# CMU-Quake/hercules

Hardware: AMD Instinct MI355X
Metric: element-updates/sec (whole node) + achieved HBM GB/s, 64M-elem box (higher is better)
Workload: dtype f64

## Files before the change

hercules_amd/capi.py:

```python
import ctypes
import os

import numpy as np

_HERE = os.path.dirname(os.path.abspath(__file__))
_LIBPATH = os.environ.get("HQ_SOLVER_LIB") or os.path.join(_HERE, "csrc", "libhq_solver.so")

HQ_VARIANT_AUTO, HQ_VARIANT_SCATTER, HQ_VARIANT_PATCH = 0, 1, 2
IPC_BLOB_BYTES = 4096

EXPORTS = ["hq_device_count", "hq_last_error", "hq_create", "hq_destroy", "hq_get_info", "hq_get_info_sized", "hq_abi_version", "hq_comm_init_ipc_n",
           "hq_options_init", "hq_create_opts", "hq_get_options", "hq_real_bytes",
           "hq_comm_unique_id", "hq_comm_init", "hq_comm_selftest", "hq_group_link", "hq_group_run", "hq_set_source", "hq_run", "hq_sync", "hq_gather", "hq_gather3",
           "hq_download", "hq_upload", "hq_phase_force", "hq_phase_update", "hq_download_force",
           "hq_run_timed", "hq_dominant_kernel", "hq_plan_check", "hq_stencil_plan_check", "hq_check_finite",
           "hq_stencil_coefficients", "hq_brick_plan_check", "hq_brick_plan_check_n", "hq_comm_init_host",
           "hq_comm_ipc_export", "hq_comm_init_ipc", "hq_comm_init_loopback",
           "hq_record_add", "hq_record_pending", "hq_record_fetch", "hq_record_clear",
           "hq_snapshot_add", "hq_snapshot_pending", "hq_snapshot_fetch", "hq_snapshot_clear",
           "hq_peak_add", "hq_peak_fetch", "hq_peak_load", "hq_peak_reset", "hq_peak_clear",
           "hq_spec_add", "hq_spec_coefficients", "hq_spec_fetch", "hq_spec_load", "hq_spec_reset", "hq_spec_clear",
           "hq_cum_add", "hq_cum_fetch", "hq_cum_load", "hq_cum_reset", "hq_cum_clear"]
HQ_SNAP_TM1, HQ_SNAP_TM2, HQ_SNAP_VEL = 1, 2, 4
HQ_PEAK_DISP, HQ_PEAK_VEL, HQ_PEAK_ACC = 1, 2, 4
HQ_SPEC_MAX_PERIODS, HQ_SPEC_NVAL = 32, 4


class HqError(RuntimeError):
    pass


HOST_EXCHANGE_FN = ctypes.CFUNCTYPE(ctypes.c_int, ctypes.c_void_p, ctypes.c_int32, ctypes.POINTER(ctypes.c_int32),
                                    ctypes.POINTER(ctypes.c_int64), ctypes.POINTER(ctypes.c_void_p), ctypes.c_int32,
                                    ctypes.POINTER(ctypes.c_int32), ctypes.POINTER(ctypes.c_int64),
                                    ctypes.POINTER(ctypes.c_void_p), ctypes.c_int32)


class _Messenger(ctypes.Structure):
    _fields_ = [("procid", ctypes.c_int32), ("nodecount", ctypes.c_int32),
                ("mapping", ctypes.c_void_p)]


class _Schedule(ctypes.Structure):
    _fields_ = [("c_count", ctypes.c_int32), ("first_c", ctypes.POINTER(_Messenger)),
                ("s_count", ctypes.c_int32), ("first_s", ctypes.POINTER(_Messenger))]


class _Desc(ctypes.Structure):
    _fields_ = [("lenum", ctypes.c_int32), ("nharbored", ctypes.c_int32), ("ldnnum", ctypes.c_int32),
# ... 37 lines not shown
                ("quantities", ctypes.c_int32), ("husid_every", ctypes.c_int32), ("husid_slots", ctypes.c_int32),
                ("reserved", ctypes.c_int32), ("threshold", ctypes.c_double * 3)]


class _Info(ctypes.Structure):
    _fields_ = [("variant", ctypes.c_int32), ("npatches", ctypes.c_int32),
                ("patch_pairs", ctypes.c_int64), ("device_bytes", ctypes.c_int64),
                ("step", ctypes.c_int32), ("nranks", ctypes.c_int32),
                ("lattice_patches", ctypes.c_int32), ("stencil_patches", ctypes.c_int32),
                ("ragged_patches", ctypes.c_int32), ("brick_units", ctypes.c_int32),
                ("brick_nodes", ctypes.c_int64), ("brick_units_pernode", ctypes.c_int32),
                ("brick_units_het", ctypes.c_int32), ("pcie_h2d_bytes", ctypes.c_int64),
                ("pcie_d2h_bytes", ctypes.c_int64), ("transport", ctypes.c_int32), ("ipc_arena_coarse", ctypes.c_int32),
                ("ipc_arena_kind", ctypes.c_int32), ("debug_halo", ctypes.c_int32),
                ("brick_units_packed", ctypes.c_int32), ("brick_units_ragged", ctypes.c_int32),
                ("brick_stream", ctypes.c_int32), ("brick_units_ragged_het", ctypes.c_int32), ("timed_steps", ctypes.c_int64),
                ("t_step_us", ctypes.c_double), ("t_shell_us", ctypes.c_double), ("t_interior_us", ctypes.c_double),
                ("t_chain_us", ctypes.c_double), ("t_chain_exposed_us", ctypes.c_double)]


OPTION_FIELDS = ["no_bricks", "brick_cz", "brick_minz", "brick_minnodes", "brick_no_het", "brick_no_ntsame", "brick_by_component",
                 "brick_stream", "brick_no_faces", "brick_half_tiles", "brick_no_pack", "patch_pipe", "patch_threads", "patch_pmax", "patch_pmerge", "patch_psplit", "patch_nlmax",
                 "patch_vmax", "patch_ragged", "patch_no_lattice", "patch_no_stencil", "patch_no_uniform", "patch_no_iso",
                 "patch_no_ntsame", "patch_no_dedup", "patch_wform", "patch_merge_rounds", "overlap", "no_overlap", "reserve_cus",
                 "cu_mask", "no_fused_share", "group_copies", "debug_halo", "ipc_arena"]


class Options(ctypes.Structure):
    _fields_ = ([("size", ctypes.c_uint64)] + [(n, ctypes.c_int32) for n in OPTION_FIELDS] +
                [("ipc_timeout_ms", ctypes.c_double), ("loopback_delay_us", ctypes.c_double),
                 ("verbose", ctypes.c_int32), ("quiet", ctypes.c_int32),
                 ("brick_ragged", ctypes.c_int32), ("brick_ragged_minfill", ctypes.c_int32),
                 ("allow_env", ctypes.c_int32), ("brick_ragged_het", ctypes.c_int32), ("reserved0", ctypes.c_int32),
                 ("phase_timing", ctypes.c_int32)])

    def __init__(self, **kw):
        super().__init__()
        load_library().hq_options_init(ctypes.byref(self), ctypes.c_uint64(ctypes.sizeof(self)))
        for k, v in kw.items():
            if k not in dict(self._fields_):
                raise TypeError("hq_options has no field %r" % k)
            setattr(self, k, v)

    def as_dict(self):
        return {k: getattr(self, k) for k, _ in self._fields_ if k != "size"}


_lib = None
_lib_f32 = None
_LIBPATH_F32 = os.environ.get("HQ_SOLVER_LIB_F32") or os.path.join(_HERE, "csrc", "libhq_solver_f32.so")


def load_library(path=None, precision="f64"):
    global _lib, _lib_f32
    if precision == "f32" and path is None:
        if _lib_f32 is None:
            _lib_f32 = load_library(_LIBPATH_F32)
            if _lib_f32.hq_real_bytes() != 4:
                raise HqError("%s was not built with -DHQ_SINGLE_PRECISION_SOLVER" % _LIBPATH_F32)
        return _lib_f32
    if _lib is not None and path is None:
        return _lib
    p = path or _LIBPATH
    if not os.path.exists(p):
        raise HqError("native library %s is missing: run `python -m hercules_amd.build` "
                      "(there is no Python/CPU fallback)" % p)
    probe = ctypes.CDLL(p, mode=ctypes.RTLD_LOCAL)
# ... 428 lines not shown
        return f


PLAN_REPORT = ("patches", "lattice_patches", "pairs", "distinct_row_blocks", "gather_passes", "gather_instructions",
               "lattice_gather_passes", "faults")


def plan_check(desc):
    rep = (ctypes.c_int64 * 8)()
    _check(load_library().hq_plan_check(ctypes.byref(desc), rep))
    return dict(zip(PLAN_REPORT, [int(v) for v in rep]))


STENCIL_PLAN_REPORT = ("patches", "tables", "full_lattices", "boundary_nodes", "corners_checked", "faults")


def stencil_plan_check(desc):
    rep = (ctypes.c_int64 * 6)()
    _check(load_library().hq_stencil_plan_check(ctypes.byref(desc), rep))
    return dict(zip(STENCIL_PLAN_REPORT, [int(v) for v in rep]))


BRICK_PLAN_REPORT = ("brick_nodes", "columns", "units", "units_one_nt_row", "het_units", "neighbours_checked",
                     "patch_nodes", "faults", "ragged_units", "ragged_nodes", "ragged_het_units", "ragged_het_nodes", "packed_units",
                     "min_unit_nx", "min_unit_ny", "min_unit_np", "ragged_min_plane_nodes", "units_one_plane_both_faces")


def brick_plan_check(desc):
    rep = (ctypes.c_int64 * len(BRICK_PLAN_REPORT))()
    _check(load_library().hq_brick_plan_check_n(ctypes.byref(desc), rep, ctypes.c_int32(len(BRICK_PLAN_REPORT))))
    return dict(zip(BRICK_PLAN_REPORT, [int(v) for v in rep]))


def comm_unique_id():
    buf = (ctypes.c_char * 128)()
    _check(load_library().hq_comm_unique_id(buf))
    return bytes(buf)


def group_link(solvers):
    arr = (ctypes.c_void_p * len(solvers))(*[s._h for s in solvers])
    lib = solvers[0]._lib
    _check(lib.hq_group_link(arr, ctypes.c_int32(len(solvers))), lib)


def group_run(solvers, nsteps):
    arr = (ctypes.c_void_p * len(solvers))(*[s._h for s in solvers])
    lib = solvers[0]._lib
    _check(lib.hq_group_run(arr, ctypes.c_int32(len(solvers)), ctypes.c_int32(nsteps)), lib)
    for s in solvers:
        s.sync()
```

hercules_amd/csrc/hq_brick.h:

```cpp
#ifndef HQ_BRICK_H
#define HQ_BRICK_H

#include <chrono>
#include <map>

#include "hq_patch.h"

#define HQ_BK_TX 64
#ifndef HQ_BK_TY
#define HQ_BK_TY 8
#endif
#define HQ_BK_THREADS (HQ_BK_TX * HQ_BK_TY)
#define HQ_BK_PY (HQ_BK_TX + 2)
#define HQ_BK_PLANE ((HQ_BK_TX + 2) * (HQ_BK_TY + 2))
#ifndef HQ_BK_ATTR
#define HQ_BK_ATTR
#endif
#define HQ_BK_NTSAME 1
#define HQ_BK_HET 2
#define HQ_BK_TOPFACE 8
#define HQ_BK_BOTFACE 16
#define HQ_BK_RAGGED 32
#define HQ_BK_PACKED 4
#ifndef HQ_BH_WAVES
#define HQ_BH_WAVES 8
#endif
#define HQ_BH_THREADS (64 * HQ_BH_WAVES)
#define HQ_BH_NRT (64 + 2 * (HQ_BH_WAVES - 1))
#define HQ_BH_TX 62
#define HQ_BH_TY (HQ_BH_WAVES - 1)
#define HQ_BH_PY 65
#define HQ_BH_CS HQ_BH_THREADS
#define HQ_BH_ROWS (65 * (HQ_BH_WAVES + 1))

struct hq_brick_unit {
    int64_t base;
    int64_t tab;
    int32_t nx, ny, np, flags;
    double  c1, c2, beta;
    double  m0, m2, m1;
    double  ft[7], fb[7];
    int64_t coef;
};

struct hq_brick_cfg {
    int cz = 32;
    int minz = 4;
    int minnodes = 512;
    int ragged = 1;
// ... 425 lines not shown
                    }
        }
        if (twice) { g_patch_err = "brick plan: a node lies in two tile columns"; return -1; }
    }
    {
        int nth = 1;
#pragma omp parallel
        {
#pragma omp single
            nth = omp_get_num_threads();
        }
        std::vector<int64_t> first((size_t)nth + 1, 0);
#pragma omp parallel for schedule(static, 1)
        for (int t = 0; t < nth; t++) {
            const int64_t lo = N * t / nth, hi = N * (t + 1) / nth;
            int64_t cnt = 0;
            for (int64_t n = lo; n < hi; n++) cnt += B->perm[(size_t)n] < 0;
            first[(size_t)t + 1] = cnt;
        }
        for (int i = 0; i < nth; i++) first[(size_t)i + 1] += first[(size_t)i];
#pragma omp parallel for schedule(static, 1)
        for (int t = 0; t < nth; t++) {
            const int64_t lo = N * t / nth, hi = N * (t + 1) / nth;
            int64_t k = nb + first[(size_t)t];
            for (int64_t n = lo; n < hi; n++) if (B->perm[(size_t)n] < 0) B->perm[(size_t)n] = (int32_t)k++;
        }
        if (nb + first[(size_t)nth] != N) { g_patch_err = "brick plan: numbering is not a permutation"; return -1; }
    }
    lap("numbering");
    B->nb = nb;
    B->ncolumns = (int32_t)cols.size();
    B->nlevels = (int32_t)levels.size();

    struct unit_t { int col; int32_t za, np; int64_t key; };
    std::vector<unit_t> us;
    int cz = cfg.cz;
    if (!hq_given(o.brick_cz)) {
        for (cz = 32; cz > 8; cz /= 2) {
            int64_t n = 0;
            for (auto& c : cols) n += (c.nz + cz - 1) / cz;
            if (n >= 512) break;
        }
    }
    for (size_t ci = 0; ci < cols.size(); ci++) {
        const column_t& c = cols[ci];
        const int32_t nch = (c.nz + cz - 1) / cz;
        const int32_t G = std::max(1, 64 / std::max(1, ntx_of_level[(size_t)c.lvl]));
        for (int32_t k = 0; k < nch; k++) {
            const int32_t za = (int32_t)((int64_t)c.nz * k / nch), zb = (int32_t)((int64_t)c.nz * (k + 1) / nch);
            const int64_t key = ((int64_t)c.lvl << 56) | ((int64_t)(c.tj / G) << 42) | ((int64_t)((c.z0 + za) / cz) << 28) |
                                ((int64_t)(c.tj % G) << 20) | (int64_t)c.ti;
            us.push_back({ (int)ci, c.z0 + za, zb - za, key });
        }
    }
    std::stable_sort(us.begin(), us.end(), [](const unit_t& a, const unit_t& b) { return a.key < b.key; });
    B->units.resize(us.size());
    std::vector<int64_t> toff(us.size() + 1, 0);
    for (size_t u = 0; u < us.size(); u++) {
        const column_t& c = cols[(size_t)us[u].col];
        const int64_t nr = 2 * (c.nx + 2) + 2 * c.ny;
        toff[u + 1] = toff[u] + ((int64_t)(us[u].np + 2) * nr + (c.rag ? us[u].np + 2 : 2) * (int64_t)c.nx * c.ny + 3) / 4 * 4;
    }
    B->tab.assign((size_t)toff[us.size()] + 64, 0);
    std::vector<int64_t> coff(us.size() + 1, 0);
    for (size_t u = 0; u < us.size(); u++)
        coff[u + 1] = coff[u] + (cols[(size_t)us[u].col].het ? (int64_t)(us[u].np + 1) * HQ_BH_THREADS * 3 : 0);
    B->coef.assign((size_t)coff[us.size()] + 8, 0.0);
    const bool try_pack = MS && MS->edata && MS->dt > 0 && !hq_set(o.brick_no_pack);
    if (try_pack) { B->coef32.assign((size_t)coff[us.size()] + 8, 0.0f); B->nt2.assign(2 * (size_t)N, 0.0); }
    int fault = 0;
    auto set_fault = [&]() {
#pragma omp atomic write
        fault = 1;
    };
    std::vector<char> same(us.size(), 0);
#pragma omp parallel for schedule(dynamic, 16)
    for (int64_t u = 0; u < (int64_t)us.size(); u++) {
        const column_t& c = cols[(size_t)us[(size_t)u].col];
        const level_t& L = levels[(size_t)c.lvl];
        const int64_t NX = L.D[0] + 1, NY = L.D[1] + 1;
        const int32_t za = us[(size_t)u].za, np = us[(size_t)u].np, nx = c.nx, ny = c.ny, nr = 2 * (nx + 2) + 2 * ny;
        auto dev = [&](int64_t X, int64_t Y, int64_t Z) -> int32_t {
            if (X < 0 || Y < 0 || Z < 0 || X > L.D[0] || Y > L.D[1] || Z > L.D[2]) { set_fault(); return 0; }
            const int32_t n = L.Ng[(size_t)((Z * NY + Y) * NX + X)];
            if (n < 0) { set_fault(); return 0; }
            return B->perm[(size_t)n];
        };
        int32_t* t = B->tab.data() + toff[(size_t)u];
// ... 202 lines not shown
    return __hiloint2double(hi, lo);
}

template <bool PERNODE, bool BYCOMP, bool RAGGED = false>
__global__ void HQ_BK_ATTR __launch_bounds__(HQ_BK_THREADS, 4)
hq_k_brick(int32_t count, int32_t per_xcd, const hq_brick_unit* __restrict__ units, const int32_t* __restrict__ tab,
           const hq_real* __restrict__ u1g, const hq_real* __restrict__ u2g, hq_real* __restrict__ ung,
           const double* __restrict__ nt3, const int32_t* __restrict__ src_ptr, const int32_t* __restrict__ src_ent,
           const double* __restrict__ F, double dt2, hq_stencil_coef sc)
{
    __shared__ __align__(16) double s_w[2 * 3 * HQ_BK_PLANE];
    const int slot = (int)(blockIdx.x & 7) * per_xcd + (int)(blockIdx.x >> 3);
    if (slot >= count) return;
    const hq_brick_unit U = units[slot];
    const int nx = U.nx, ny = U.ny, np = U.np, nxy = nx * ny, nr = 2 * (nx + 2) + 2 * ny;
    const int t = threadIdx.x, lx = t & (HQ_BK_TX - 1), ly = t >> 6;
    const bool active = lx < nx && ly < ny;
    const int sidx = active ? ly * nx + lx : 0;
    const int myrow = (ly + 1) * HQ_BK_PY + lx + 1;
    const bool ring = t < nr;
    int rrow;
    {
        int rx, ry;
        if (t < nx + 2) { rx = t - 1; ry = -1; }
        else if (t < 2 * (nx + 2)) { rx = t - (nx + 2) - 1; ry = ny; }
        else if (t < 2 * (nx + 2) + ny) { rx = -1; ry = t - 2 * (nx + 2); }
        else { rx = nx; ry = t - 2 * (nx + 2) - ny; }
        rrow = (ry + 1) * HQ_BK_PY + rx + 1;
    }
    const int32_t* __restrict__ utab = tab + U.tab;
    const int rofs = ring ? t : 0;
    const int32_t* __restrict__ cap = utab + (int64_t)(np + 2) * nr;
    int32_t vOut = -1, vMid = RAGGED ? cap[sidx] : 0, vCur = RAGGED ? cap[nxy + sidx] : 0, vNext = 0;
    const int32_t id_lo = RAGGED ? (vMid >= 0 ? vMid : -vMid - 2) : cap[sidx];
    const double beta = U.beta;
    double P[6], Q[2];
#pragma unroll
    for (int i = 0; i < 6; i++) P[i] = hq_uniform(U.c1 * sc.p1[i] + U.c2 * sc.p2[i]);
#pragma unroll
    for (int i = 0; i < 2; i++) Q[i] = hq_uniform(U.c1 * sc.q1[i] + U.c2 * sc.q2[i]);
    const bool has_src = F && src_ptr[slot + 1] > src_ptr[slot];

    hq_real x1[3] = { 0, 0, 0 }, x2[3] = { 0, 0, 0 }, y1[3] = { 0, 0, 0 }, y2[3] = { 0, 0, 0 };
    double mn[3] = { U.m0, U.m2, U.m1 };
    double m0A = hq_uniform(1.0 / U.m0), m0B = m0A;
    double fA[3] = { 0.0, 0.0, 0.0 }, fB[3] = { 0.0, 0.0, 0.0 };
    int32_t rid = utab[rofs];

#define HQ_BK_LOAD(node_)                                                                             \
    {                                                                                                 \
        const int64_t a_ = (node_);                                                                   \
        if (active && (!RAGGED || a_ >= 0)) {                                                         \
            _Pragma("unroll") for (int d = 0; d < 3; d++) { x1[d] = u1g[3 * a_ + d]; x2[d] = u2g[3 * a_ + d]; } \
            if (PERNODE) { _Pragma("unroll") for (int d = 0; d < 3; d++) mn[d] = nt3[3 * a_ + d]; }    \
        }                                                                                             \
        if (ring && (!RAGGED || rid >= 0)) {                                                          \
            const int64_t b_ = (int64_t)rid;                                                          \
            _Pragma("unroll") for (int d = 0; d < 3; d++) { y1[d] = u1g[3 * b_ + d]; y2[d] = u2g[3 * b_ + d]; } \
        }                                                                                             \
    }
#define HQ_BK_PUT(s_, acc_, M2_, M1_)                                                                 \
    {                                                                                                 \
        hq_lds_double* img_ = (hq_lds_double*)s_w + 3 * HQ_BK_PLANE * (s_);                            \
        if (active) {                                                                                 \
            _Pragma("unroll") for (int d = 0; d < 3; d++) {                                           \
                const double a1_ = x1[d], a2_ = x2[d];                                                \
                img_[3 * myrow + d] = a1_ + beta * (a1_ - a2_);                                       \
                acc_[d] += (M2_) * a1_ - (M1_) * a2_;                                                 \
            }                                                                                         \
        }                                                                                             \
        if (ring) { _Pragma("unroll") for (int d = 0; d < 3; d++) { const double b1_ = y1[d], b2_ = y2[d]; img_[3 * rrow + d] = b1_ + beta * (b1_ - b2_); } } \
    }

    const bool topf = !PERNODE && !RAGGED && (U.flags & HQ_BK_TOPFACE) != 0, botf = !PERNODE && !RAGGED && (U.flags & HQ_BK_BOTFACE) != 0;
    const double rho = hq_uniform((U.c1 - U.c2) / (U.c1 + U.c2));

    HQ_BK_LOAD((int64_t)id_lo)
    rid = utab[nr + rofs];
    if (topf) HQ_BK_PUT(0, fB, U.ft[1 + d], U.ft[4 + d])
    else { double dummy[3] = { 0.0, 0.0, 0.0 }; HQ_BK_PUT(0, dummy, mn[1], mn[2]) }
    for (int k = 0; k <= np + 1; k++) {
        if (k <= np) {
            if (RAGGED) {
                HQ_BK_LOAD((int64_t)(vCur >= 0 ? vCur : -vCur - 2))
                if (k < np) vNext = cap[(k + 2) * nxy + sidx];
            } else HQ_BK_LOAD(k == np ? (int64_t)cap[nxy + sidx] : U.base + (int64_t)k * nxy + sidx)
            if (k < np) rid = utab[(k + 2) * nr + rofs];
        }
        __syncthreads();
        const hq_lds_double* __restrict__ q = (const hq_lds_double*)s_w + 3 * (HQ_BK_PLANE * (k & 1) + myrow);
        double m[3], g[3], Uo[3];
        if (BYCOMP) {
            double A_x, A_y;
            {
                const double C = q[2], XM = q[2 - 3], XP = q[2 + 3], YM = q[2 - 3 * HQ_BK_PY], YP = q[2 + 3 * HQ_BK_PY];
                const double MM = q[2 - 3 * HQ_BK_PY - 3], PM = q[2 - 3 * HQ_BK_PY + 3], MP = q[2 + 3 * HQ_BK_PY - 3], PP = q[2 + 3 * HQ_BK_PY + 3];
                const double sxy = (XM + XP) + (YM + YP), dg = (MM + PP) + (PM + MP);
                m[2] = fma(P[0], C, fma(P[2], sxy, P[4] * dg));
                g[2] = fma(P[1], C, fma(P[3], sxy, P[5] * dg));
                Uo[0] = fma(Q[0], XP - XM, Q[1] * ((PP - MP) + (PM - MM)));
                Uo[1] = fma(Q[0], YP - YM, Q[1] * ((PP - PM) + (MP - MM)));
            }
            __builtin_amdgcn_sched_barrier(0);
            {
                const double C = q[0], XM = q[0 - 3], XP = q[0 + 3], YM = q[0 - 3 * HQ_BK_PY], YP = q[0 + 3 * HQ_BK_PY];
                const double MM = q[0 - 3 * HQ_BK_PY - 3], PM = q[0 - 3 * HQ_BK_PY + 3], MP = q[0 + 3 * HQ_BK_PY - 3], PP = q[0 + 3 * HQ_BK_PY + 3];
                const double sx = XM + XP, sy = YM + YP, dg = (MM + PP) + (PM + MP);
                A_x = (PP + MM) - (PM + MP);
                m[0] = fma(P[0], C, fma(P[1], sx, fma(P[2], sy, P[3] * dg)));
                g[0] = fma(P[2], C, fma(P[3], sx, fma(P[4], sy, P[5] * dg)));
                Uo[2] = fma(Q[0], XP - XM, Q[1] * ((PP - MP) + (PM - MM)));
            }
            __builtin_amdgcn_sched_barrier(0);
            {
                const double C = q[1], XM = q[1 - 3], XP = q[1 + 3], YM = q[1 - 3 * HQ_BK_PY], YP = q[1 + 3 * HQ_BK_PY];
                const double MM = q[1 - 3 * HQ_BK_PY - 3], PM = q[1 - 3 * HQ_BK_PY + 3], MP = q[1 + 3 * HQ_BK_PY - 3], PP = q[1 + 3 * HQ_BK_PY + 3];
                const double sx = XM + XP, sy = YM + YP, dg = (MM + PP) + (PM + MP);
                A_y = (PP + MM) - (PM + MP);
                m[1] = fma(P[0], C, fma(P[1], sy, fma(P[2], sx, fma(P[3], dg, Q[0] * A_x))));
                g[1] = fma(P[2], C, fma(P[3], sy, fma(P[4], sx, fma(P[5], dg, Q[1] * A_x))));
// ... 387 lines not shown
```

hercules_amd/csrc/hq_opts.h:

```cpp
#ifndef HQ_OPTS_H
#define HQ_OPTS_H

#include <cstddef>
#include <cstdlib>
#include <cstring>

struct hq_opt_entry { const char* env; size_t off; int kind; };

#define HQ_OPT_I(env_, field_) { env_, offsetof(hq_options, field_), 0 }
#define HQ_OPT_D(env_, field_) { env_, offsetof(hq_options, field_), 1 }
static const hq_opt_entry g_opt_table[] = {
    HQ_OPT_I("HQ_NO_BRICKS", no_bricks), HQ_OPT_I("HQ_BRICK_CZ", brick_cz), HQ_OPT_I("HQ_BRICK_MINZ", brick_minz),
    HQ_OPT_I("HQ_BRICK_MINNODES", brick_minnodes), HQ_OPT_I("HQ_BRICK_NO_HET", brick_no_het),
    HQ_OPT_I("HQ_BRICK_NO_NTSAME", brick_no_ntsame), HQ_OPT_I("HQ_BRICK_BY_COMPONENT", brick_by_component),
    HQ_OPT_I("HQ_BRICK_STREAM", brick_stream), HQ_OPT_I("HQ_BRICK_NO_FACES", brick_no_faces), HQ_OPT_I("HQ_BRICK_HALF_TILES", brick_half_tiles), HQ_OPT_I("HQ_BRICK_NO_PACK", brick_no_pack), HQ_OPT_I("HQ_PATCH_PIPE", patch_pipe), HQ_OPT_I("HQ_PATCH_THREADS", patch_threads),
    HQ_OPT_I("HQ_PATCH_PMAX", patch_pmax), HQ_OPT_I("HQ_PATCH_PMERGE", patch_pmerge), HQ_OPT_I("HQ_PATCH_PSPLIT", patch_psplit),
    HQ_OPT_I("HQ_PATCH_NLMAX", patch_nlmax), HQ_OPT_I("HQ_PATCH_VMAX", patch_vmax), HQ_OPT_I("HQ_PATCH_RAGGED", patch_ragged),
    HQ_OPT_I("HQ_PATCH_NO_LATTICE", patch_no_lattice), HQ_OPT_I("HQ_PATCH_NO_STENCIL", patch_no_stencil),
    HQ_OPT_I("HQ_PATCH_NO_UNIFORM", patch_no_uniform), HQ_OPT_I("HQ_PATCH_NO_ISO", patch_no_iso),
    HQ_OPT_I("HQ_PATCH_NO_NTSAME", patch_no_ntsame), HQ_OPT_I("HQ_PATCH_NO_DEDUP", patch_no_dedup),
    HQ_OPT_I("HQ_PATCH_WFORM", patch_wform), HQ_OPT_I("HQ_PATCH_MERGE_ROUNDS", patch_merge_rounds),
    HQ_OPT_I("HQ_OVERLAP", overlap), HQ_OPT_I("HQ_NO_OVERLAP", no_overlap), HQ_OPT_I("HQ_RESERVE_CUS", reserve_cus),
    HQ_OPT_I("HQ_CU_MASK", cu_mask), HQ_OPT_I("HQ_NO_FUSED_SHARE", no_fused_share), HQ_OPT_I("HQ_GROUP_COPIES", group_copies),
    HQ_OPT_I("HQ_DEBUG_HALO", debug_halo), HQ_OPT_I("HQ_IPC_ARENA", ipc_arena), HQ_OPT_D("HQ_IPC_TIMEOUT_MS", ipc_timeout_ms),
    HQ_OPT_D("HQ_LOOPBACK_DELAY_US", loopback_delay_us), HQ_OPT_I("HQ_PATCH_VERBOSE", verbose), HQ_OPT_I("HQ_QUIET", quiet),
    HQ_OPT_I("HQ_BRICK_RAGGED", brick_ragged), HQ_OPT_I("HQ_BRICK_RAGGED_MINFILL", brick_ragged_minfill),
    HQ_OPT_I("HQ_PHASE_TIMING", phase_timing), HQ_OPT_I("HQ_BRICK_RAGGED_HET", brick_ragged_het),
};
#undef HQ_OPT_I
#undef HQ_OPT_D

static void hq_options_defaults(hq_options* o)
{
    o->size = sizeof(hq_options);
    for (const hq_opt_entry& e : g_opt_table) {
        if (e.kind == 0) *(int32_t*)((char*)o + e.off) = -1;
        else *(double*)((char*)o + e.off) = -1.0;
    }
    o->allow_env = -1;
    o->reserved0 = -1;
}

static void hq_options_adopt(hq_options* dst, const hq_options* src)
{
    hq_options_defaults(dst);
    if (!src) return;
    const size_t n = (size_t)(src->size < sizeof(hq_options) ? src->size : sizeof(hq_options));
    if (n > sizeof(uint64_t)) memcpy((char*)dst + sizeof(uint64_t), (const char*)src + sizeof(uint64_t), n - sizeof(uint64_t));
    dst->size = sizeof(hq_options);
}

static int hq_opt_env_int(const char* env, const char* v)
{
    if (!strcmp(env, "HQ_IPC_ARENA")) return !strcmp(v, "fine") ? 0 : (!strcmp(v, "uncached") ? 1 : (!strcmp(v, "coarse") ? 2 : atoi(v)));
    if (!*v) return 1;
    return atoi(v);
}

static void hq_options_resolve(hq_options* out, const hq_options* caller)
{
// ... 24 lines not shown
```

hercules_amd/csrc/hq_plan_check.h:

```cpp
#ifndef HQ_PLAN_CHECK_H
#define HQ_PLAN_CHECK_H

extern "C" int hq_plan_check(const hq_desc* d, int64_t report[8])
{
    hq_options opts;
    hq_options_resolve(&opts, nullptr);
    if (!report) return hq_fail(HQ_ERR_ARG, "inconsistent mesh description%s", "");
    hq_prep prep;
    HQ_TRY(hq_prepare(d, opts, 0, &prep));
    const int64_t E = d->lenum, N = d->nharbored;
    const hq_dangling& dn = prep.dn;
    bool want_lattice = false;
    const hq_patch_cfg cfg = hq_patch_cfg_of(opts, dn.n > 0, d->node_xyz != nullptr, &want_lattice);
    hq_patch_host H;
    if (hq_patch_plan_host(opts, cfg, E, N, d->lnid, d->node_xyz, dn, want_lattice, &H) != 0)
        return hq_fail(HQ_ERR_ARG, "patch plan: %s", hq_patch_error());
    const hq_lattice_tab& T = hq_lattice();
    int64_t nlat = 0, passes = 0, lpasses = 0, instr = 0, bad = 0;
    std::vector<int32_t> covered((size_t)N, 0);
#pragma omp parallel for schedule(dynamic, 64) reduction(+ : nlat, passes, lpasses, instr, bad)
    for (int64_t p = 0; p < (int64_t)H.desc.size(); p++) {
        const hq_patch_desc& D = H.desc[(size_t)p];
        const bool lat = H.lattice[(size_t)p] != 0;
        nlat += lat;
// ... 367 lines not shown
    report[0] = B.nb; report[1] = B.ncolumns; report[2] = (int64_t)B.units.size(); report[3] = nsame;
    report[4] = B.nhet + B.nrhet; report[5] = nchecked; report[6] = N - B.nb; report[7] = bad;
    report[8] = B.nrag; report[10] = B.nrhet; report[12] = B.npacked + B.nrpacked;
    report[13] = report[14] = report[15] = INT64_MAX;
    for (const hq_brick_unit& U : B.units) {
        report[13] = std::min<int64_t>(report[13], U.nx); report[14] = std::min<int64_t>(report[14], U.ny);
        report[15] = std::min<int64_t>(report[15], U.np);
        report[17] += U.np == 1 && (U.flags & HQ_BK_TOPFACE) && (U.flags & HQ_BK_BOTFACE);
        if (!(U.flags & HQ_BK_RAGGED)) continue;
        const int64_t nxy = (int64_t)U.nx * U.ny;
        const int32_t* pl = B.tab.data() + U.tab + (int64_t)(U.np + 2) * (2 * (U.nx + 2) + 2 * U.ny);
        for (int64_t k = 1; k <= U.np; k++) {
            int64_t own = 0;
            for (int64_t i = k * nxy; i < (k + 1) * nxy; i++) own += pl[i] >= 0;
            report[(U.flags & HQ_BK_HET) ? 11 : 9] += own;
            report[16] = report[16] ? std::min(report[16], own) : own;
        }
    }
    if (bad) return hq_fail(HQ_ERR_STATE, "brick plan self-check failed%s", "");
    return HQ_OK;
}

extern "C" int hq_brick_plan_check(const hq_desc* d, int64_t report[8]) { return hq_brick_plan_check_n(d, report, 8); }

extern "C" int hq_brick_plan_check_n(const hq_desc* d, int64_t* report, int32_t n)
{
    int64_t r[HQ_BRICK_REPORT_N];
    if (!report || n < 8) return hq_fail(HQ_ERR_ARG, "hq_brick_plan_check_n: a report of at least 8 entries%s", "");
    const int rc = hq_brick_plan_check_impl(d, r);
    for (int k = 0; k < n; k++) report[k] = k < HQ_BRICK_REPORT_N ? r[k] : 0;
    return rc;
}

#endif
```

hercules_amd/host.py:

```python
import ctypes
import os

import numpy as np

from . import capi

_HERE = os.path.dirname(os.path.abspath(__file__))
_LIBPATH = os.environ.get("HQ_HOST_LIB") or os.path.join(_HERE, "csrc", "libhq_host.so")

DAMPING = {"none": 0, "rayleigh": 1, "mass": 2}
EXPORTS = ["hqh_box_create", "hqh_box_destroy", "hqh_box_get_info", "hqh_box_desc", "hqh_box_lnid",
           "hqh_box_node_ijk", "hqh_box_etable", "hqh_box_ntable", "hqh_box_owner", "hqh_box_material", "hqh_ntable_to_float",
           "hqh_point_source", "hqh_stations", "hqh_solver_run", "hqh_source_table",
           "hqh_forcefile_info", "hqh_forcefile_read", "hqh_forcefile_write",
           "hqh_solver_run_on", "hqh_solver_run_async", "hqh_checkpoint_write_fields", "hqh_wavefield_write_block",
           "hqh_checkpoint_write", "hqh_checkpoint_read", "hqh_station_format", "hqh_station_format_derivs",
           "hqh_station_kinematics", "hqh_peak_fold", "hqh_cum_fold", "hqh_husid_cross", "hqh_sdof_coef", "hqh_spec_fold", "hqh_station_header", "hqh_wavefield_create", "hqh_wavefield_write",
           "hqh_octbox_create", "hqh_octbox_destroy", "hqh_octbox_desc", "hqh_octbox_view",
           "hqh_cvm_open", "hqh_cvm_close", "hqh_cvm_info", "hqh_cvm_query", "hqh_cvm_grid"]


class _BoxParams(ctypes.Structure):
    _fields_ = [("nx", ctypes.c_int32), ("ny", ctypes.c_int32), ("nz", ctypes.c_int32),
                ("h", ctypes.c_double), ("nlayers", ctypes.c_int32),
# ... 213 lines not shown
        return out

    def schedule(self):
        d = capi._Desc()
        self._lib.hqh_box_desc(self._h, ctypes.byref(d))
        out = {}
        for key, cnt, first in (("c", d.an_sched.c_count, d.an_sched.first_c),
                                ("s", d.an_sched.s_count, d.an_sched.first_s)):
            out[key] = [(first[i].procid,
                         _view(first[i].mapping, (first[i].nodecount,), np.int32).copy()) for i in range(cnt)]
        return out

    def plan_check(self):
        d = capi._Desc()
        rc = self._lib.hqh_box_desc(self._h, ctypes.byref(d))
        if rc != 0:
            raise capi.HqError("hqh_box_desc failed: %d" % rc)
        return capi.plan_check(d)

    def stencil_plan_check(self):
        d = capi._Desc()
        rc = self._lib.hqh_box_desc(self._h, ctypes.byref(d))
        if rc != 0:
            raise capi.HqError("hqh_box_desc failed: %d" % rc)
        return capi.stencil_plan_check(d)

    def brick_plan_check(self):
        d = capi._Desc()
        rc = self._lib.hqh_box_desc(self._h, ctypes.byref(d))
        if rc != 0:
            raise capi.HqError("hqh_box_desc failed: %d" % rc)
        return capi.brick_plan_check(d)

    def create_solver(self, variant=capi.HQ_VARIANT_AUTO, device=0, tm1=None, tm2=None, options=None, precision="f64"):
        d = capi._Desc()
        rc = self._lib.hqh_box_desc(self._h, ctypes.byref(d))
        if rc != 0:
            raise capi.HqError("hqh_box_desc failed: %d" % rc)
        return _solver_from_desc(d, self.ntable, variant, device, tm1, tm2, options, precision)

    def point_source(self, x, y, z, strike=0.0, dip=90.0, rake=0.0):
        n = ctypes.c_int32()
        ids = np.zeros(8, np.int32)
        pat = np.zeros((8, 3))
        rc = self._lib.hqh_point_source(self._h, ctypes.c_double(x), ctypes.c_double(y), ctypes.c_double(z),
                                        ctypes.c_double(strike), ctypes.c_double(dip), ctypes.c_double(rake),
                                        ctypes.byref(n), ids.ctypes.data_as(ctypes.c_void_p),
                                        pat.ctypes.data_as(ctypes.c_void_p))
        if rc != 0:
            raise capi.HqError("hqh_point_source failed: %d" % rc)
        return (ids, pat) if n.value == 8 else (ids[:0], pat[:0])

    def stations(self, xyz):
        xyz = np.ascontiguousarray(xyz, np.float64).reshape(-1, 3)
        n = len(xyz)
        ids = np.zeros((n, 8), np.int32)
        phi = np.zeros((n, 8))
        mine = np.zeros(n, np.int32)
        rc = self._lib.hqh_stations(self._h, ctypes.c_int32(n), xyz.ctypes.data_as(ctypes.c_void_p),
                                    ids.ctypes.data_as(ctypes.c_void_p), phi.ctypes.data_as(ctypes.c_void_p),
                                    mine.ctypes.data_as(ctypes.c_void_p))
        if rc != 0:
            raise capi.HqError("hqh_stations failed: %d" % rc)
        return ids, phi, mine

    def run_params(self, *args, **kw):
# ... 170 lines not shown
                                   _view(first[i].mapping, (first[i].nodecount,), np.int32).copy())
                                  for i in range(cnt)]
        return out

    def close(self):
        if getattr(self, "_h", None) and self._h.value:
            self.lnid = self.node_xyz = self.dangling = self.etable = self.ntable = self.owner = self.gid = None
            self._lib.hqh_octbox_destroy(self._h)
            self._h = ctypes.c_void_p()

    __del__ = close

    def plan_check(self):
        d = capi._Desc()
        rc = self._lib.hqh_octbox_desc(self._h, ctypes.byref(d))
        if rc != 0:
            raise capi.HqError("hqh_octbox_desc failed: %d" % rc)
        return capi.plan_check(d)

    def stencil_plan_check(self):
        d = capi._Desc()
        rc = self._lib.hqh_octbox_desc(self._h, ctypes.byref(d))
        if rc != 0:
            raise capi.HqError("hqh_octbox_desc failed: %d" % rc)
        return capi.stencil_plan_check(d)

    def brick_plan_check(self):
        d = capi._Desc()
        rc = self._lib.hqh_octbox_desc(self._h, ctypes.byref(d))
        if rc != 0:
            raise capi.HqError("hqh_octbox_desc failed: %d" % rc)
        return capi.brick_plan_check(d)

    def create_solver(self, variant=capi.HQ_VARIANT_AUTO, device=0, tm1=None, tm2=None, options=None, precision="f64"):
        d = capi._Desc()
        rc = self._lib.hqh_octbox_desc(self._h, ctypes.byref(d))
        if rc != 0:
            raise capi.HqError("hqh_octbox_desc failed: %d" % rc)
        return _solver_from_desc(d, self.ntable, variant, device, tm1, tm2, options, precision)


def _solver_from_desc(d, ntable, variant, device, tm1, tm2, options, precision):
    d.variant = variant
    real = np.float32 if precision == "f32" else np.float64
    keep = []
    if precision == "f32":
        nt = np.empty(ntable.shape, np.float32)
        src = np.ascontiguousarray(ntable, np.float64)
        rc = load_library().hqh_ntable_to_float(src.ctypes.data_as(ctypes.c_void_p), ctypes.c_int64(len(src)),
                                                nt.ctypes.data_as(ctypes.c_void_p))
        if rc != 0:
            raise capi.HqError("hqh_ntable_to_float failed: %d" % rc)
        keep.append(nt)
        d.nTable = nt.ctypes.data
    for name, a in (("tm1", tm1), ("tm2", tm2)):
        if a is not None:
            a = np.ascontiguousarray(a, real)
            keep.append(a)
            setattr(d, name, a.ctypes.data)
    s = capi.Solver.__new__(capi.Solver)
    s._lib = capi.load_library(precision=precision)
    s.real = real
    s._h = ctypes.c_void_p()
    s._trackers = capi._no_trackers()
    s.N, s.E = d.nharbored, d.lenum
    if isinstance(options, dict):
# ... 294 lines not shown
```

include/hq_solver.h:

```cpp
#ifndef HQ_SOLVER_H
#define HQ_SOLVER_H

#include <stdint.h>

#ifdef __cplusplus
extern "C" {
#endif

#define HQ_API __attribute__((visibility("default")))

typedef struct hq_ctx hq_ctx;

typedef enum {
    HQ_OK            =  0,
    HQ_ERR_ARG       = -1,
    HQ_ERR_NOMEM     = -2,
    HQ_ERR_DEVICE    = -3,
    HQ_ERR_NODEVICE  = -4,
    HQ_ERR_COMM      = -5,
    HQ_ERR_STATE     = -6
} hq_status;

enum {
    HQ_VARIANT_AUTO    = 0,
// ... 101 lines not shown
    int32_t patch_threads;
    int32_t patch_pmax;
    int32_t patch_pmerge;
    int32_t patch_psplit;
    int32_t patch_nlmax;
    int32_t patch_vmax;
    int32_t patch_ragged;
    int32_t patch_no_lattice;
    int32_t patch_no_stencil;
    int32_t patch_no_uniform;
    int32_t patch_no_iso;
    int32_t patch_no_ntsame;
    int32_t patch_no_dedup;
    int32_t patch_wform;
    int32_t patch_merge_rounds;
    int32_t overlap;
    int32_t no_overlap;
    int32_t reserve_cus;
    int32_t cu_mask;
    int32_t no_fused_share;
    int32_t group_copies;
    int32_t debug_halo;
    int32_t ipc_arena;
    double  ipc_timeout_ms;
    double  loopback_delay_us;
    int32_t verbose;
    int32_t quiet;
    int32_t brick_ragged;
    int32_t brick_ragged_minfill;
    int32_t allow_env;
    int32_t brick_ragged_het;
    int32_t reserved0;
    int32_t phase_timing;
} hq_options;

HQ_API void hq_options_init(hq_options* opts, uint64_t size);
HQ_API int  hq_create_opts(const hq_desc* desc, int device, const hq_options* opts, hq_ctx** out);
HQ_API int  hq_get_options(hq_ctx* ctx, hq_options* out, uint64_t size);

HQ_API int hq_destroy(hq_ctx* ctx);

#define HQ_ABI_VERSION 6
HQ_API int hq_abi_version(void);
HQ_API int hq_real_bytes(void);
HQ_API int hq_get_info_sized(hq_ctx* ctx, hq_info* info, uint64_t size);
HQ_API int hq_get_info(hq_ctx* ctx, hq_info* info);
#ifndef HQ_SOLVER_IMPLEMENTATION
#define hq_get_info(ctx, info) hq_get_info_sized((ctx), (info), (uint64_t)sizeof(hq_info))
#endif

HQ_API int hq_comm_unique_id(void* id128);
HQ_API int hq_comm_init(hq_ctx* ctx, const void* id128);
HQ_API int hq_comm_selftest(hq_ctx* ctx, int32_t count);

typedef int (*hq_host_exchange_fn)(void* user, int32_t nrecv, const int32_t* recv_peer, const int64_t* recv_count,
                                   double* const* recv_buf, int32_t nsend, const int32_t* send_peer,
                                   const int64_t* send_count, const double* const* send_buf, int32_t tag);
HQ_API int hq_comm_init_host(hq_ctx* ctx, hq_host_exchange_fn fn, void* user);

#define HQ_IPC_BLOB_BYTES 4096
HQ_API int hq_comm_ipc_export(hq_ctx* ctx, void* blob);
HQ_API int hq_comm_init_ipc(hq_ctx* ctx, const void* all_blobs);
HQ_API int hq_comm_init_ipc_n(hq_ctx* ctx, const void* all_blobs, int32_t nblobs);
HQ_API int hq_comm_init_loopback(hq_ctx* ctx);

HQ_API int hq_group_link(hq_ctx** ctxs, int32_t n);
// ... 77 lines not shown
HQ_API int hq_spec_clear(hq_ctx* ctx);

typedef struct {
    int32_t        npoints;
    int32_t        nodes_per_point;
    const int32_t* ids;
    const double*  phi;
    int32_t        rate, first_step;
    int32_t        quantities;
    int32_t        husid_every, husid_slots;
    int32_t        reserved;
    double         threshold[3];
} hq_cum_desc;
HQ_API int hq_cum_add(hq_ctx* ctx, const hq_cum_desc* desc, int32_t* handle);
HQ_API int hq_cum_fetch(hq_ctx* ctx, int32_t handle, double* sums, int32_t* span, double* curve, int32_t* curve_steps,
                        int32_t* nfilled, int64_t* nsamples);
HQ_API int hq_cum_load(hq_ctx* ctx, int32_t handle, const double* sums, const int32_t* span, const double* curve,
                       const int32_t* curve_steps, int32_t nfilled, int64_t nsamples);
HQ_API int hq_cum_reset(hq_ctx* ctx, int32_t handle);
HQ_API int hq_cum_clear(hq_ctx* ctx);

HQ_API int hq_phase_force(hq_ctx* ctx);
HQ_API int hq_phase_update(hq_ctx* ctx);
HQ_API int hq_download_force(hq_ctx* ctx, double* force);

HQ_API int hq_run_timed(hq_ctx* ctx, int32_t nsteps, double* total_ms, double* kernel_ms_avg);

HQ_API int hq_plan_check(const hq_desc* desc, int64_t report[8]);

HQ_API int hq_stencil_plan_check(const hq_desc* desc, int64_t report[6]);

HQ_API int hq_brick_plan_check(const hq_desc* desc, int64_t report[8]);
HQ_API int hq_brick_plan_check_n(const hq_desc* desc, int64_t* report, int32_t n);

HQ_API int hq_stencil_coefficients(double out[16]);

HQ_API const char* hq_dominant_kernel(hq_ctx* ctx);

#ifdef __cplusplus
}
#endif
#endif
```

Before: 66.83 billion.

## Reorder brick units into column slabs with selectable intra-slab ordering

Changes how brick units are sorted and numbered. Columns are now grouped into slabs of W tiles (4 by default) across and 64/W down, then by z chunk. Within each slab an order option picks the traversal: row, column, serpentine or Morton. The default replaces the old wide-row grouping, so node numbering and neighbour locality in memory change, aiming for better cache reuse of the ring/cap neighbour loads. The diff also adds experiment-only ablation macros in the kernel, a plan-introspection API, and new options, none of which are active by default.

```diff
diff --git a/hercules_amd/capi.py b/hercules_amd/capi.py
--- a/hercules_amd/capi.py
+++ b/hercules_amd/capi.py
@@ -14,7 +14,7 @@
            "hq_comm_unique_id", "hq_comm_init", "hq_comm_selftest", "hq_group_link", "hq_group_run", "hq_set_source", "hq_run", "hq_sync", "hq_gather", "hq_gather3",
            "hq_download", "hq_upload", "hq_phase_force", "hq_phase_update", "hq_download_force",
            "hq_run_timed", "hq_dominant_kernel", "hq_plan_check", "hq_stencil_plan_check", "hq_check_finite",
-           "hq_stencil_coefficients", "hq_brick_plan_check", "hq_brick_plan_check_n", "hq_comm_init_host",
+           "hq_stencil_coefficients", "hq_brick_plan_check", "hq_brick_plan_check_n", "hq_brick_plan_units", "hq_comm_init_host",
            "hq_comm_ipc_export", "hq_comm_init_ipc", "hq_comm_init_loopback",
            "hq_record_add", "hq_record_pending", "hq_record_fetch", "hq_record_clear",
            "hq_snapshot_add", "hq_snapshot_pending", "hq_snapshot_fetch", "hq_snapshot_clear",
@@ -118,7 +118,7 @@
                  ("verbose", ctypes.c_int32), ("quiet", ctypes.c_int32),
                  ("brick_ragged", ctypes.c_int32), ("brick_ragged_minfill", ctypes.c_int32),
                  ("allow_env", ctypes.c_int32), ("brick_ragged_het", ctypes.c_int32), ("reserved0", ctypes.c_int32),
-                 ("phase_timing", ctypes.c_int32)])
+                 ("phase_timing", ctypes.c_int32), ("brick_order", ctypes.c_int32), ("brick_slab_cols", ctypes.c_int32)])
 
     def __init__(self, **kw):
         super().__init__()
@@ -613,6 +613,18 @@
     return dict(zip(BRICK_PLAN_REPORT, [int(v) for v in rep]))
 
 
+def brick_plan_units(desc, options=None):
+    lib = load_library()
+    opts = Options(**options) if isinstance(options, dict) else options
+    po = ctypes.byref(opts) if opts is not None else None
+    n = ctypes.c_int64(0)
+    perm = np.empty(int(desc.nharbored), dtype=np.int32)
+    _check(lib.hq_brick_plan_units(ctypes.byref(desc), po, ctypes.c_int64(0), ctypes.byref(n), None, _ptr(perm)))
+    units = np.zeros((int(n.value), 5), dtype=np.int64)
+    _check(lib.hq_brick_plan_units(ctypes.byref(desc), po, ctypes.c_int64(len(units)), ctypes.byref(n), _ptr_or_pad(units), None))
+    return units, perm
+
+
 def comm_unique_id():
     buf = (ctypes.c_char * 128)()
     _check(load_library().hq_comm_unique_id(buf))
diff --git a/hercules_amd/csrc/hq_brick.h b/hercules_amd/csrc/hq_brick.h
--- a/hercules_amd/csrc/hq_brick.h
+++ b/hercules_amd/csrc/hq_brick.h
@@ -15,6 +15,18 @@
 #define HQ_BK_PLANE ((HQ_BK_TX + 2) * (HQ_BK_TY + 2))
 #ifndef HQ_BK_ATTR
 #define HQ_BK_ATTR
+#endif
+#define HQ_BK_ORDER_DEFAULT 0
+#define HQ_BK_SLAB_COLS_DEFAULT 4
+#ifndef HQ_BK_ABL
+#define HQ_BK_ABL 0
+#elif !defined(HQ_EXPERIMENT)
+#error "HQ_BK_ABL is for experiment builds (-DHQ_EXPERIMENT)"
+#endif
+#if HQ_BK_ABL == 2
+#define HQ_BK_CAP_HI (U.base + (int64_t)(np - 1) * nxy + sidx)
+#else
+#define HQ_BK_CAP_HI ((int64_t)cap[nxy + sidx])
 #endif
 #define HQ_BK_NTSAME 1
 #define HQ_BK_HET 2
@@ -506,8 +518,10 @@
     B->ncolumns = (int32_t)cols.size();
     B->nlevels = (int32_t)levels.size();
 
-    struct unit_t { int col; int32_t za, np; int64_t key; };
+    struct unit_t { int col; int32_t za, np; int64_t key, in; };
     std::vector<unit_t> us;
+    const int order = std::min(3, std::max(0, hq_value_or(o.brick_order, HQ_BK_ORDER_DEFAULT)));
+    auto spread = [](int64_t v) { int64_t r = 0; for (int b = 0; b < 16; b++) r |= ((v >> b) & 1) << (2 * b); return r; };
     int cz = cfg.cz;
     if (!hq_given(o.brick_cz)) {
         for (cz = 32; cz > 8; cz /= 2) {
@@ -519,15 +533,19 @@
     for (size_t ci = 0; ci < cols.size(); ci++) {
         const column_t& c = cols[ci];
         const int32_t nch = (c.nz + cz - 1) / cz;
-        const int32_t G = std::max(1, 64 / std::max(1, ntx_of_level[(size_t)c.lvl]));
+        const int32_t ntx = std::max(1, ntx_of_level[(size_t)c.lvl]);
+        const int32_t W = std::min(ntx, hq_set(o.brick_slab_cols) ? o.brick_slab_cols : HQ_BK_SLAB_COLS_DEFAULT), nsc = (ntx + W - 1) / W;
+        const int32_t G = std::max(1, 64 / W);
+        const int64_t slab = (int64_t)(c.tj / G) * nsc + c.ti / W, li = c.ti % W, lj = c.tj % G;
+        const int64_t in = order == 0 ? (lj << 20) | li : (order == 1 ? (li << 20) | lj : (order == 2 ? (li << 20) | ((li & 1) ? G - 1 - lj : lj) :
+                                                                                          (spread(lj) << 1) | spread(li)));
         for (int32_t k = 0; k < nch; k++) {
             const int32_t za = (int32_t)((int64_t)c.nz * k / nch), zb = (int32_t)((int64_t)c.nz * (k + 1) / nch);
-            const int64_t key = ((int64_t)c.lvl << 56) | ((int64_t)(c.tj / G) << 42) | ((int64_t)((c.z0 + za) / cz) << 28) |
-                                ((int64_t)(c.tj % G) << 20) | (int64_t)c.ti;
-            us.push_back({ (int)ci, c.z0 + za, zb - za, key });
-        }
-    }
-    std::stable_sort(us.begin(), us.end(), [](const unit_t& a, const unit_t& b) { return a.key < b.key; });
+            const int64_t key = ((int64_t)c.lvl << 56) | (slab << 28) | (int64_t)((c.z0 + za) / cz);
+            us.push_back({ (int)ci, c.z0 + za, zb - za, key, in });
+        }
+    }
+    std::stable_sort(us.begin(), us.end(), [](const unit_t& a, const unit_t& b) { return a.key != b.key ? a.key < b.key : a.in < b.in; });
     B->units.resize(us.size());
     std::vector<int64_t> toff(us.size() + 1, 0);
     for (size_t u = 0; u < us.size(); u++) {
@@ -796,7 +814,7 @@
     const int rofs = ring ? t : 0;
     const int32_t* __restrict__ cap = utab + (int64_t)(np + 2) * nr;
     int32_t vOut = -1, vMid = RAGGED ? cap[sidx] : 0, vCur = RAGGED ? cap[nxy + sidx] : 0, vNext = 0;
-    const int32_t id_lo = RAGGED ? (vMid >= 0 ? vMid : -vMid - 2) : cap[sidx];
+    const int32_t id_lo = RAGGED ? (vMid >= 0 ? vMid : -vMid - 2) : (HQ_BK_ABL == 2 ? (int32_t)U.base + sidx : cap[sidx]);
     const double beta = U.beta;
     double P[6], Q[2];
 #pragma unroll
@@ -809,7 +827,7 @@
     double mn[3] = { U.m0, U.m2, U.m1 };
     double m0A = hq_uniform(1.0 / U.m0), m0B = m0A;
     double fA[3] = { 0.0, 0.0, 0.0 }, fB[3] = { 0.0, 0.0, 0.0 };
-    int32_t rid = utab[rofs];
+    int32_t rid = HQ_BK_ABL == 3 ? 0 : utab[rofs];
 
 #define HQ_BK_LOAD(node_)                                                                             \
     {                                                                                                 \
@@ -818,8 +836,8 @@
             _Pragma("unroll") for (int d = 0; d < 3; d++) { x1[d] = u1g[3 * a_ + d]; x2[d] = u2g[3 * a_ + d]; } \
             if (PERNODE) { _Pragma("unroll") for (int d = 0; d < 3; d++) mn[d] = nt3[3 * a_ + d]; }    \
         }                                                                                             \
-        if (ring && (!RAGGED || rid >= 0)) {                                                          \
-            const int64_t b_ = (int64_t)rid;                                                          \
+        const int64_t b_ = HQ_BK_ABL == 3 ? a_ : (int64_t)rid;                                        \
+        if (HQ_BK_ABL != 1 && ring && (!RAGGED || b_ >= 0)) {                                         \
             _Pragma("unroll") for (int d = 0; d < 3; d++) { y1[d] = u1g[3 * b_ + d]; y2[d] = u2g[3 * b_ + d]; } \
         }                                                                                             \
     }
@@ -840,7 +858,7 @@
     const double rho = hq_uniform((U.c1 - U.c2) / (U.c1 + U.c2));
 
     HQ_BK_LOAD((int64_t)id_lo)
-    rid = utab[nr + rofs];
+    if (HQ_BK_ABL != 3) rid = utab[nr + rofs];
     if (topf) HQ_BK_PUT(0, fB, U.ft[1 + d], U.ft[4 + d])
     else { double dummy[3] = { 0.0, 0.0, 0.0 }; HQ_BK_PUT(0, dummy, mn[1], mn[2]) }
     for (int k = 0; k <= np + 1; k++) {
@@ -848,8 +866,8 @@
             if (RAGGED) {
                 HQ_BK_LOAD((int64_t)(vCur >= 0 ? vCur : -vCur - 2))
                 if (k < np) vNext = cap[(k + 2) * nxy + sidx];
-            } else HQ_BK_LOAD(k == np ? (int64_t)cap[nxy + sidx] : U.base + (int64_t)k * nxy + sidx)
-            if (k < np) rid = utab[(k + 2) * nr + rofs];
+            } else HQ_BK_LOAD(k == np ? HQ_BK_CAP_HI : U.base + (int64_t)k * nxy + sidx)
+            if (HQ_BK_ABL != 3 && k < np) rid = utab[(k + 2) * nr + rofs];
         }
         __syncthreads();
         const hq_lds_double* __restrict__ q = (const hq_lds_double*)s_w + 3 * (HQ_BK_PLANE * (k & 1) + myrow);
diff --git a/hercules_amd/csrc/hq_opts.h b/hercules_amd/csrc/hq_opts.h
--- a/hercules_amd/csrc/hq_opts.h
+++ b/hercules_amd/csrc/hq_opts.h
@@ -26,6 +26,7 @@
     HQ_OPT_D("HQ_LOOPBACK_DELAY_US", loopback_delay_us), HQ_OPT_I("HQ_PATCH_VERBOSE", verbose), HQ_OPT_I("HQ_QUIET", quiet),
     HQ_OPT_I("HQ_BRICK_RAGGED", brick_ragged), HQ_OPT_I("HQ_BRICK_RAGGED_MINFILL", brick_ragged_minfill),
     HQ_OPT_I("HQ_PHASE_TIMING", phase_timing), HQ_OPT_I("HQ_BRICK_RAGGED_HET", brick_ragged_het),
+    HQ_OPT_I("HQ_BRICK_ORDER", brick_order), HQ_OPT_I("HQ_BRICK_SLAB_COLS", brick_slab_cols),
 };
 #undef HQ_OPT_I
 #undef HQ_OPT_D
diff --git a/hercules_amd/csrc/hq_plan_check.h b/hercules_amd/csrc/hq_plan_check.h
--- a/hercules_amd/csrc/hq_plan_check.h
+++ b/hercules_amd/csrc/hq_plan_check.h
@@ -423,4 +423,25 @@
     return rc;
 }
 
+extern "C" int hq_brick_plan_units(const hq_desc* d, const hq_options* o, int64_t cap, int64_t* nunits, int64_t* units, int32_t* perm)
+{
+    if (!d || !nunits || !d->node_xyz || !d->eTable || !d->nTable || (cap > 0 && !units))
+        return hq_fail(HQ_ERR_ARG, "inconsistent mesh description (node_xyz is needed)%s", "");
+    if (o && o->size < sizeof(uint64_t)) return hq_fail(HQ_ERR_ARG, "hq_options.size is not set (hq_options_init)%s", "");
+    hq_options opts;
+    hq_options_resolve(&opts, o);
+    hq_prep prep;
+    HQ_TRY(hq_prepare(d, opts, HQ_PREP_BRICKS, &prep));
+    const hq_brick_host& B = prep.bricks;
+    *nunits = (int64_t)B.units.size();
+    for (int64_t u = 0; u < *nunits && u < cap; u++) {
+        const hq_brick_unit& U = B.units[(size_t)u];
+        int64_t* r = units + 5 * u;
+        r[0] = U.base; r[1] = U.nx; r[2] = U.ny; r[3] = U.np; r[4] = U.flags;
+    }
+    if (perm)
+        for (int64_t n = 0; n < d->nharbored; n++) perm[n] = prep.perm.empty() ? (int32_t)n : prep.perm[(size_t)n];
+    return HQ_OK;
+}
+
 #endif
diff --git a/hercules_amd/host.py b/hercules_amd/host.py
--- a/hercules_amd/host.py
+++ b/hercules_amd/host.py
@@ -269,6 +269,13 @@
             raise capi.HqError("hqh_box_desc failed: %d" % rc)
         return capi.brick_plan_check(d)
 
+    def brick_plan_units(self, options=None):
+        d = capi._Desc()
+        rc = self._lib.hqh_box_desc(self._h, ctypes.byref(d))
+        if rc != 0:
+            raise capi.HqError("hqh_box_desc failed: %d" % rc)
+        return capi.brick_plan_units(d, options)
+
     def create_solver(self, variant=capi.HQ_VARIANT_AUTO, device=0, tm1=None, tm2=None, options=None, precision="f64"):
         d = capi._Desc()
         rc = self._lib.hqh_box_desc(self._h, ctypes.byref(d))
@@ -505,6 +512,13 @@
             raise capi.HqError("hqh_octbox_desc failed: %d" % rc)
         return capi.brick_plan_check(d)
 
+    def brick_plan_units(self, options=None):
+        d = capi._Desc()
+        rc = self._lib.hqh_octbox_desc(self._h, ctypes.byref(d))
+        if rc != 0:
+            raise capi.HqError("hqh_octbox_desc failed: %d" % rc)
+        return capi.brick_plan_units(d, options)
+
     def create_solver(self, variant=capi.HQ_VARIANT_AUTO, device=0, tm1=None, tm2=None, options=None, precision="f64"):
         d = capi._Desc()
         rc = self._lib.hqh_octbox_desc(self._h, ctypes.byref(d))
diff --git a/include/hq_solver.h b/include/hq_solver.h
--- a/include/hq_solver.h
+++ b/include/hq_solver.h
@@ -157,6 +157,8 @@
     int32_t brick_ragged_het;
     int32_t reserved0;
     int32_t phase_timing;
+    int32_t brick_order;
+    int32_t brick_slab_cols;
 } hq_options;
 
 HQ_API void hq_options_init(hq_options* opts, uint64_t size);
@@ -300,6 +302,7 @@
 
 HQ_API int hq_brick_plan_check(const hq_desc* desc, int64_t report[8]);
 HQ_API int hq_brick_plan_check_n(const hq_desc* desc, int64_t* report, int32_t n);
+HQ_API int hq_brick_plan_units(const hq_desc* desc, const hq_options* opts, int64_t cap, int64_t* nunits, int64_t* units, int32_t* perm);
 
 HQ_API int hq_stencil_coefficients(double out[16]);
 
```

Result: no change. 66.36 billion (-0.7%).
